# HansiZeng/scaling-retriever

Hardware: AMD Instinct MI355X
Metric: MSMARCO-Dev queries/sec end-to-end (query encode + dense brute-force top-1000) (higher is better)
Workload: dtype f32

## Files before the change

### scaling_retriever_amd/csrc/attention_f32.hip

```cpp
#include "kernels.h"
#include <math.h>

#define AF_KC 64
#define AF_RPW 4
#define AF_ROWS 16

template <int HD>
__global__ __launch_bounds__(256) void attention_f32_kernel(AttnF32Args a) {
    constexpr int DPL = HD / 64;
    __shared__ float Ks[AF_KC][HD + 1];
    __shared__ float qs[AF_ROWS][HD];
    __shared__ float ps[AF_ROWS][AF_KC];
    __shared__ unsigned char kval[AF_KC];
    const int b = blockIdx.x, h = blockIdx.y;
    const int tid = threadIdx.x, lane = tid & 63, wave = tid >> 6;
    const int t0 = a.cu_seqlens[b];
    const int S = a.cu_seqlens[b + 1] - t0;
    const int r0 = blockIdx.z * AF_ROWS;
    if (r0 >= S || S <= a.only_gt) return;
    const int G = a.nh / a.nkv, kvh = h / G;
    const int ld = (a.nh + 2 * a.nkv) * HD;
    const int koff = a.nh * HD + kvh * HD, voff = (a.nh + a.nkv) * HD + kvh * HD;
    const int nrows = (S - r0) < AF_ROWS ? (S - r0) : AF_ROWS;

// ... 102 lines not shown
#pragma unroll
            for (int e = 0; e < DPL; ++e) o[r][e] = 0.f;
        }
        for (int k0 = 0; k0 < S; k0 += AF_KC) {
            const int nk = (S - k0) < AF_KC ? (S - k0) : AF_KC;
            __syncthreads();
            for (int i = tid; i < nk * HD; i += 64 * G) {
                const int k = i / HD, d = i % HD;
                Ks[k][d] = a.qkv[(int64_t)(t0 + k0 + k) * ld + koff + d];
                if constexpr (V_LDS) Vs[k][d] = a.qkv[(int64_t)(t0 + k0 + k) * ld + voff + d];
            }
            if (tid < AF_KC) kval[tid] = (tid < nk) ? a.key_valid[t0 + k0 + tid] : 0;
            __syncthreads();
            const bool valid = kval[lane] != 0;
#pragma unroll
            for (int r = 0; r < AF_RPW; ++r) {
                const int row = rq + r;
                if (row >= nrows) break;
#pragma unroll
                for (int e = 0; e < DPL; ++e) qs[wave][lane + 64 * e] = a.qkv[(int64_t)(t0 + r0 + row) * ld + h * HD + lane + 64 * e];
                __builtin_amdgcn_wave_barrier();
                float s = 0.f;
                for (int d = 0; d < HD; ++d) s += qs[wave][d] * Ks[lane][d];
                s = valid ? s * a.scale : -INFINITY;
                float mx = s;
                for (int off = 32; off > 0; off >>= 1) mx = fmaxf(mx, __shfl_xor(mx, off));
                if (mx == -INFINITY) continue;
                const float m_new = fmaxf(m[r], mx);
                const float corr = expf(m[r] - m_new);
                const float p = valid ? expf(s - m_new) : 0.f;
                float sum = p;
                for (int off = 32; off > 0; off >>= 1) sum += __shfl_xor(sum, off);
                l[r] = l[r] * corr + sum;
                m[r] = m_new;
                ps[wave][lane] = p;
                __builtin_amdgcn_wave_barrier();
                float acc[DPL];
#pragma unroll
                for (int e = 0; e < DPL; ++e) acc[e] = 0.f;
                for (int k = 0; k < nk; ++k) {
                    const float pk = ps[wave][k];
                    if constexpr (V_LDS) {
                        acc[0] += pk * Vs[k][lane];
                    } else {
                        const float* vrow = a.qkv + (int64_t)(t0 + k0 + k) * ld + voff;
#pragma unroll
                        for (int e = 0; e < DPL; ++e) acc[e] += pk * vrow[lane + 64 * e];
                    }
                }
#pragma unroll
                for (int e = 0; e < DPL; ++e) o[r][e] = o[r][e] * corr + acc[e];
            }
        }
#pragma unroll
        for (int r = 0; r < AF_RPW; ++r) {
            const int row = rq + r;
            if (row >= nrows) break;
            const float inv = l[r] > 0.f ? 1.0f / l[r] : 0.f;
            if (a.out_f32) {
#pragma unroll
                for (int e = 0; e < DPL; ++e) a.out_f32[(int64_t)(t0 + r0 + row) * a.nh * HD + h * HD + lane + 64 * e] = o[r][e] * inv;
                continue;
            }
            bf16_t* orow = a.out + (int64_t)(t0 + r0 + row) * ldo;
#pragma unroll
            for (int e = 0; e < DPL; ++e) {
                unsigned short p[3];
                split_bf16x3(o[r][e] * inv, p[0], p[1], p[2]);
                const int col = h * HD + lane + 64 * e;
                for (int sg = 0; sg < a.out_map.n_seg; ++sg) orow[(int64_t)sg * a.nh * HD + col] = p[a.out_map.plane[sg]];
            }
        }
    }
}

template <int HD>
__global__ __launch_bounds__(256) void attention_f32_mfma_kernel(AttnF32Args a) {
    constexpr int LDK = HD + 1, CB = HD / 16;
    extern __shared__ float af_smem[];
    const int b = blockIdx.x, kvh = blockIdx.y;
    const int tid = threadIdx.x, lane = tid & 63, wave = tid >> 6;
    const int t0 = a.cu_seqlens[b];
    const int S = a.cu_seqlens[b + 1] - t0;
    if (S <= 0 || S > a.only_le) return;
    const int nkb = (S + 15) >> 4;
    const int SP = nkb * 16;
    float* Ks = af_smem;
    float* Vs = Ks + SP * LDK;
    float* Qs = Vs + SP * LDK + wave * 16 * LDK;
    const int G = a.nh / a.nkv;
    const int h = kvh * G + wave;
    const int ld = (a.nh + 2 * a.nkv) * HD;
    const int koff = a.nh * HD + kvh * HD, voff = (a.nh + a.nkv) * HD + kvh * HD;
    for (int i = tid; i < SP * (HD / 4); i += 256) {
        const int k = i / (HD / 4), d = (i % (HD / 4)) * 4;
        f32x4 kv = {0.f, 0.f, 0.f, 0.f}, vv = {0.f, 0.f, 0.f, 0.f};
        if (k < S) {
            kv = *reinterpret_cast<const f32x4*>(a.qkv + (int64_t)(t0 + k) * ld + koff + d);
            vv = *reinterpret_cast<const f32x4*>(a.qkv + (int64_t)(t0 + k) * ld + voff + d);
        }
#pragma unroll
        for (int e = 0; e < 4; ++e) { Ks[k * LDK + d + e] = kv[e]; Vs[k * LDK + d + e] = vv[e]; }
    }
    const int g = lane >> 4, c = lane & 15;
    unsigned vmask = 0;
    for (int kb = 0; kb < nkb; ++kb)
#pragma unroll
        for (int r = 0; r < 4; ++r) {
            const int key = 16 * kb + 4 * g + r;
            if (key < S && a.key_valid[t0 + key]) vmask |= 1u << (4 * kb + r);
        }
    __syncthreads();
    const int64_t ldo = (int64_t)a.out_map.n_seg * a.nh * HD;
    for (int qb = 0; qb < nkb; ++qb) {
        for (int i = lane; i < 16 * (HD / 4); i += 64) {
            const int r = i / (HD / 4), d = (i % (HD / 4)) * 4;
            f32x4 qv = {0.f, 0.f, 0.f, 0.f};
            if (16 * qb + r < S) qv = *reinterpret_cast<const f32x4*>(a.qkv + (int64_t)(t0 + 16 * qb + r) * ld + h * HD + d);
#pragma unroll
            for (int e = 0; e < 4; ++e) Qs[r * LDK + d + e] = qv[e];
        }
        __builtin_amdgcn_fence(__ATOMIC_ACQ_REL, "wavefront");
        f32x4 st[4];
        float qf[HD / 4];
#pragma unroll
        for (int kk = 0; kk < HD / 4; ++kk) qf[kk] = Qs[c * LDK + 4 * kk + g];
#pragma unroll
        for (int kb = 0; kb < 4; ++kb) {
            st[kb] = f32x4{0.f, 0.f, 0.f, 0.f};
            if (kb < nkb) {
#pragma unroll
                for (int kk = 0; kk < HD / 4; ++kk)
                    st[kb] = __builtin_amdgcn_mfma_f32_16x16x4f32(Ks[(16 * kb + c) * LDK + 4 * kk + g], qf[kk], st[kb], 0, 0, 0);
            }
        }
        float m = -INFINITY;
#pragma unroll
        for (int kb = 0; kb < 4; ++kb)
#pragma unroll
            for (int r = 0; r < 4; ++r) {
                const bool v = (vmask >> (4 * kb + r)) & 1;
                st[kb][r] = v ? st[kb][r] * a.scale : -INFINITY;
                m = fmaxf(m, st[kb][r]);
            }
        m = fmaxf(m, __shfl_xor(m, 16));
        m = fmaxf(m, __shfl_xor(m, 32));
        float sum = 0.f;
#pragma unroll
        for (int kb = 0; kb < 4; ++kb)
#pragma unroll
            for (int r = 0; r < 4; ++r) {
                const float p = (m > -INFINITY && st[kb][r] > -INFINITY) ? expf(st[kb][r] - m) : 0.f;
                st[kb][r] = p;
                sum += p;
            }
        sum += __shfl_xor(sum, 16);
        sum += __shfl_xor(sum, 32);
        const float inv = sum > 0.f ? 1.0f / sum : 0.f;
#pragma unroll
        for (int kb = 0; kb < 4; ++kb)
#pragma unroll
            for (int r = 0; r < 4; ++r) st[kb][r] *= inv;
#pragma unroll
        for (int cb = 0; cb < CB; ++cb) {
            f32x4 o = {0.f, 0.f, 0.f, 0.f};
#pragma unroll
            for (int kb = 0; kb < 4; ++kb) {
                if (kb < nkb) {
#pragma unroll
                    for (int mm = 0; mm < 4; ++mm)
                        o = __builtin_amdgcn_mfma_f32_16x16x4f32(st[kb][mm], Vs[(16 * kb + 4 * g + mm) * LDK + 16 * cb + c], o, 0, 0, 0);
                }
            }
#pragma unroll
            for (int r = 0; r < 4; ++r) {
                const int row = 16 * qb + 4 * g + r;
                if (row >= S) continue;
                const int col = h * HD + 16 * cb + c;
                if (a.out_f32) {
                    a.out_f32[(int64_t)(t0 + row) * a.nh * HD + col] = o[r];
                } else {
                    unsigned short p[3];
                    split_bf16x3(o[r], p[0], p[1], p[2]);
                    bf16_t* orow = a.out + (int64_t)(t0 + row) * ldo;
                    for (int sg = 0; sg < a.out_map.n_seg; ++sg) orow[(int64_t)sg * a.nh * HD + col] = p[a.out_map.plane[sg]];
                }
            }
        }
    }
}

template <int HD>
static int launch_attention_f32_mfma(const AttnF32Args& a, hipStream_t s) {
    const int sp = (int)ceil_div64(a.max_seqlen < 64 ? a.max_seqlen : 64, 16) * 16;
    const size_t lds = sizeof(float) * (size_t)(2 * sp + 4 * 16) * (HD + 1);
    static DeviceOnce attr_once;
    if (bool* slot = attr_once.pending()) {
        SR_CHECK_HIP(hipFuncSetAttribute(reinterpret_cast<const void*>(&attention_f32_mfma_kernel<HD>),
                                         hipFuncAttributeMaxDynamicSharedMemorySize, (int)(sizeof(float) * (2 * 64 + 64) * (HD + 1))));
        *slot = true;
    }
    const dim3 grid((unsigned)a.B, (unsigned)a.nkv), block(256);
    SR_REQUIRE(grid.y <= 65535, "attention(fp32): grid too large");
    hipLaunchKernelGGL(attention_f32_mfma_kernel<HD>, grid, block, lds, s, a);
    SR_CHECK_LAUNCH();
    return SR_OK;
}

int launch_attention_f32(const AttnF32Args& a_in, hipStream_t s) {
    AttnF32Args a = a_in;
    SR_REQUIRE(a.nh % a.nkv == 0, "attention(fp32): num_heads %d not a multiple of num_kv_heads %d", a.nh, a.nkv);
    SR_REQUIRE(a.out_f32 || (a.out_map.n_seg >= 1 && a.out_map.n_seg <= SR_MAX_SEG), "attention(fp32): bad segment map");
    if (a.B == 0 || a.max_seqlen <= 0) return SR_OK;
    const int G = a.nh / a.nkv;
    a.only_le = 0; a.only_gt = 0;
    const char* env_m = sr_dev_getenv("SR_ATTN_F32_MFMA");
    if (G == 4 && (a.hd == 64 || a.hd == 128) && !(env_m && *env_m == '0')) {
        a.only_le = 64;
        SR_TRY(a.hd == 64 ? launch_attention_f32_mfma<64>(a, s) : launch_attention_f32_mfma<128>(a, s));
        if (a.max_seqlen <= 64) return SR_OK;
        a.only_le = 0; a.only_gt = 64;
    }
    const char* env = sr_dev_getenv("SR_ATTN_F32_GQA");
    if (G == 4 && !(env && *env == '0')) {
        const dim3 grid((unsigned)a.B, (unsigned)a.nkv, (unsigned)ceil_div64(a.max_seqlen, AF_ROWS)), block(256);
        SR_REQUIRE(grid.y <= 65535 && grid.z <= 65535, "attention(fp32): grid too large");
        switch (a.hd) {
            case 64: hipLaunchKernelGGL((attention_f32_gqa_kernel<64, 4>), grid, block, 0, s, a); break;
            case 128: hipLaunchKernelGGL((attention_f32_gqa_kernel<128, 4>), grid, block, 0, s, a); break;
            default: sr_set_error("attention(fp32): head_dim %d not supported (64 or 128)", a.hd); return SR_ERR_UNSUPPORTED;
        }
        SR_CHECK_LAUNCH();
        return SR_OK;
    }
    const dim3 grid((unsigned)a.B, (unsigned)a.nh, (unsigned)ceil_div64(a.max_seqlen, AF_ROWS)), block(256);
    SR_REQUIRE(grid.y <= 65535 && grid.z <= 65535, "attention(fp32): grid too large");
    switch (a.hd) {
        case 64: hipLaunchKernelGGL(attention_f32_kernel<64>, grid, block, 0, s, a); break;
        case 128: hipLaunchKernelGGL(attention_f32_kernel<128>, grid, block, 0, s, a); break;
        default: sr_set_error("attention(fp32): head_dim %d not supported (64 or 128)", a.hd); return SR_ERR_UNSUPPORTED;
    }
    SR_CHECK_LAUNCH();
    return SR_OK;
}
```

### scaling_retriever_amd/csrc/encoder.hip

```cpp
#include "kernels.h"
#include <math.h>
#include <mutex>
#include <string>
#include <vector>

__global__ void plan_rows_kernel(const int64_t* __restrict__ mask, int B, int L, int mode, int* __restrict__ span_start,
                                 int* __restrict__ span_len, int* __restrict__ pool_start, int* __restrict__ row_len,
                                 const int* __restrict__ row_shift) {
    const int b = blockIdx.x;
    const int lane = threadIdx.x;
    int len = 0, first = L, last = -1;
    for (int p = lane; p < L; p += 64) {
        if (mask[(int64_t)b * L + p] != 0) {
            ++len;
            first = p < first ? p : first;
            last = p > last ? p : last;
        }
    }
    for (int off = 32; off > 0; off >>= 1) {
        len += __shfl_xor(len, off);
        const int f = __shfl_xor(first, off), l = __shfl_xor(last, off);
        first = f < first ? f : first;
        last = l > last ? l : last;
    }
// ... 861 lines not shown
    }
    SR_CHECK_HIP(hipDeviceSynchronize());
    m->finalized = true;
    return SR_OK;
}

extern "C" int sr_model_weight_segments(sr_model* m, int32_t* out, int64_t capacity, int64_t* n) {
    SR_REQUIRE(m && n, "sr_model_weight_segments: null argument");
    SR_REQUIRE(m->finalized, "sr_model_weight_segments: sr_model_finalize was not called");
    const sr_model_config& c = m->cfg;
    std::vector<int32_t> v;
    const bool f16p = c.fp32_planes == SR_FP32_PLANES_F16;
    const int32_t plain = c.fp32_planes ? split_map_w(c.fp32_planes).n_seg : 0;
    for (const LayerW& l : m->layers) {
        v.push_back(f16p ? l.qkv_seg : plain); v.push_back(f16p ? l.o_seg : plain);
        v.push_back(f16p ? l.gu_seg : plain); v.push_back(f16p ? l.down_seg : plain);
    }
    if (c.has_lm_head) v.push_back(f16p ? m->lm_head_seg : plain);
    *n = (int64_t)v.size();
    SR_REQUIRE(capacity >= 0 && (capacity == 0 || out), "sr_model_weight_segments: bad output buffer");
    for (int64_t i = 0; i < capacity && i < (int64_t)v.size(); ++i) out[i] = v[(size_t)i];
    return SR_OK;
}

enum { PREC_BF16 = 0, PREC_FP32 = 1 };

static int ensure_fp32_workspace(sr_model* m) {
    if (m->xs) return SR_OK;
    const sr_model_config& c = m->cfg;
    SR_REQUIRE(c.fp32_planes > 0, "encode(fp32): the model was created with fp32_planes = 0 (bf16 regime only)");
    const int64_t Tm = m->Tm, H = c.hidden_size, I = c.intermediate_size;
    const int64_t nq = (int64_t)c.num_heads * c.head_dim, nkv = (int64_t)c.num_kv_heads * c.head_dim;
    const int64_t nsg = split_map_a(c.fp32_planes).n_seg;
    auto A = [&](void** p, int64_t bytes) {
        if (hipMalloc(p, (size_t)bytes) != hipSuccess) { *p = nullptr; return false; }
        return hipMemset(*p, 0, (size_t)bytes) == hipSuccess;
    };
    const bool f16p = c.fp32_planes == SR_FP32_PLANES_F16;
    bool ok = A((void**)&m->xs, Tm * H * 2 * nsg) && A((void**)&m->qkv_f, Tm * (nq + 2 * nkv) * 4) &&
              A((void**)&m->attn_s, Tm * nq * 2 * nsg) && A((void**)&m->act_s, Tm * I * 2 * nsg);
    if (ok && f16p)
        ok = A((void**)&m->attn_f, Tm * nq * 4) && A((void**)&m->act_f, Tm * I * 4) && A((void**)&m->xs_i, Tm * 4) &&
             A((void**)&m->attn_i, Tm * 4) && A((void**)&m->act_i, Tm * 4) && A((void**)&m->act_sc, Tm * 4);
    if (!ok) {
        auto F = [](void* p) { if (p) (void)hipFree(p); };
        F(m->xs); F(m->qkv_f); F(m->attn_s); F(m->act_s); F(m->attn_f); F(m->act_f); F(m->xs_i); F(m->attn_i); F(m->act_i);
        m->xs = nullptr; m->qkv_f = nullptr; m->attn_s = nullptr; m->act_s = nullptr;
        m->attn_f = nullptr; m->act_f = nullptr; m->xs_i = nullptr; m->attn_i = nullptr; m->act_i = nullptr;
        sr_set_error("encode(fp32): hipMalloc of the fp32-regime workspace failed (%lld tokens)", (long long)Tm);
        return SR_ERR_NOMEM;
    }
    return SR_OK;
}

static int launch_rmsnorm_split(float* x, const float* embed, const int* tok_id, const float* w, bf16_t* xs, int T, int H,
                                float eps, const SplitMap& map, hipStream_t s) {
    if (T == 0) return SR_OK;
    hipLaunchKernelGGL(rmsnorm_split_kernel, dim3((unsigned)ceil_div64(T, 4)), dim3(256), 0, s, x, embed, tok_id, w, xs, T, H, eps,
                       map);
    SR_CHECK_LAUNCH();
    return SR_OK;
}

static int model_forward(sr_model* m, const int64_t* d_ids, const int64_t* d_mask, int B, int L, int mode, int prec,
                         hipStream_t s, int* T_out, const int32_t* d_shift = nullptr) {
    const sr_model_config& c = m->cfg;
    SR_REQUIRE(m->finalized, "encode: sr_model_finalize was not called");
    SR_REQUIRE(B >= 1 && L >= 1, "encode: bad batch shape [%d, %d]", B, L);
    SR_REQUIRE(B <= m->Bm, "encode: batch of %d sequences exceeds max_batch_seqs %d", B, m->Bm);
    SR_REQUIRE(L <= m->max_pos, "encode: sequence length %d exceeds %d", L, m->max_pos);
    SR_REQUIRE(d_ids && d_mask, "encode: null input");
    if (prec == PREC_FP32) SR_TRY(ensure_fp32_workspace(m));
    const int H = c.hidden_size, I = c.intermediate_size;
    const int nq = c.num_heads * c.head_dim, nkv = c.num_kv_heads * c.head_dim;

    hipLaunchKernelGGL(plan_rows_kernel, dim3(B), dim3(64), 0, s, d_mask, B, L, mode, m->span_start, m->span_len,
                       m->pool_start, m->row_len, d_shift);
    hipLaunchKernelGGL(plan_scan_kernel, dim3(1), dim3(256), 0, s, m->span_len, B, m->cu);
    SR_CHECK_LAUNCH();
    SR_CHECK_HIP(hipMemcpyAsync(m->h_cu, m->cu, (size_t)(B + 1) * 4, hipMemcpyDeviceToHost, s));
    SR_CHECK_HIP(hipStreamSynchronize(s));
    const int T = m->h_cu[B];
    int max_len = 0;
    for (int b = 0; b < B; ++b) max_len = (m->h_cu[b + 1] - m->h_cu[b]) > max_len ? (m->h_cu[b + 1] - m->h_cu[b]) : max_len;
    SR_REQUIRE(T <= m->Tm, "encode: batch packs to %d tokens, workspace holds %d (raise max_batch_tokens or split the batch)", T, m->Tm);
    *T_out = T;
    m->last_T = T;
    if (T == 0) return SR_OK;
    hipLaunchKernelGGL(plan_tokens_kernel, dim3(B), dim3(128), 0, s, d_ids, d_mask, L, m->span_start, m->cu, m->tok_id,
                       m->pos, m->key_valid, m->seq_of, c.vocab_size, mode, d_shift);
    SR_CHECK_LAUNCH();

    if (prec == PREC_FP32 && c.fp32_planes == SR_FP32_PLANES_F16) {
        auto split_rows = [&](float* src, const float* embed, const int* tok, const float* w, bf16_t* dst, float* inv, int K, int nseg) {
            launch_rows_split_h(src, embed, tok, w, dst, inv, T, K, c.rms_norm_eps, nseg, s);
        };
        const char* env_fa = sr_dev_getenv("SR_FP32_FUSED_ACT");
        const bool fused_act = m->layers[0].gu_cmax && !(env_fa && *env_fa == '0');
        for (int li = 0; li < c.num_layers; ++li) {
            LayerW& l = m->layers[li];
            split_rows(m->x, li == 0 ? m->embed : (const float*)nullptr, li == 0 ? m->tok_id : (const int*)nullptr, l.ln1, m->xs, m->xs_i, H,
                       l.qkv_seg);
            GemmArgs g{};
            g.A = m->xs; g.W = l.wqkv_s; g.M = T; g.N = nq + 2 * nkv; g.K = l.qkv_seg * H; g.C = m->qkv_f; g.a_scale = m->xs_i; g.w_scale = l.wqkv_i;
            g.pos = m->pos; g.rope_cos = m->rope_cos; g.rope_sin = m->rope_sin; g.n_rope = nq + nkv; g.head_dim = c.head_dim;
            SR_TRY(launch_gemm_bf16(EPI_QKV_ROPE_F32_H, g, s));
            AttnF32Args a{};
            a.qkv = m->qkv_f; a.out_f32 = m->attn_f; a.out = nullptr; a.cu_seqlens = m->cu; a.key_valid = m->key_valid;
            a.B = B; a.nh = c.num_heads; a.nkv = c.num_kv_heads; a.hd = c.head_dim;
            a.scale = 1.0f / sqrtf((float)c.head_dim); a.max_seqlen = max_len;
            SR_TRY(launch_attention_f32(a, s));
            split_rows(m->attn_f, nullptr, nullptr, nullptr, m->attn_s, m->attn_i, nq, l.o_seg);
            g = GemmArgs{};
            g.A = m->attn_s; g.W = l.wo_s; g.M = T; g.N = H; g.K = l.o_seg * nq; g.C = m->x; g.a_scale = m->attn_i; g.w_scale = l.wo_i;
            SR_TRY(launch_gemm_bf16(EPI_RESID_F32_H, g, s));
            if (fused_act) {
                launch_rows_split_h(m->x, nullptr, nullptr, l.ln2, m->xs, m->xs_i, T, H, c.rms_norm_eps, l.gu_seg, s, l.gu_cmax, m->act_sc,
                                    m->act_i);
                g = GemmArgs{};
                g.A = m->xs; g.W = l.wgu_s; g.M = T; g.N = 2 * I; g.K = l.gu_seg * H; g.C = m->act_s; g.a_scale = m->xs_i; g.w_scale = l.wgu_i;
                g.out_scale = m->act_sc; g.out_nseg = l.down_seg;
                SR_TRY(launch_gemm_bf16(EPI_SWIGLU_SPLIT_H, g, s));
            } else {
                split_rows(m->x, nullptr, nullptr, l.ln2, m->xs, m->xs_i, H, l.gu_seg);
                g = GemmArgs{};
                g.A = m->xs; g.W = l.wgu_s; g.M = T; g.N = 2 * I; g.K = l.gu_seg * H; g.C = m->act_f; g.a_scale = m->xs_i; g.w_scale = l.wgu_i;
                SR_TRY(launch_gemm_bf16(EPI_SWIGLU_F32_H, g, s));
                split_rows(m->act_f, nullptr, nullptr, nullptr, m->act_s, m->act_i, I, l.down_seg);
            }
            g = GemmArgs{};
            g.A = m->act_s; g.W = l.wdown_s; g.M = T; g.N = H; g.K = l.down_seg * I; g.C = m->x; g.a_scale = m->act_i; g.w_scale = l.wdown_i;
            SR_TRY(launch_gemm_bf16(EPI_RESID_F32_H, g, s));
        }
        SR_CHECK_LAUNCH();
        return SR_OK;
    }
    if (prec == PREC_FP32) {
        const SplitMap ma = split_map_a(c.fp32_planes);
        const int nsg = ma.n_seg;
        for (int li = 0; li < c.num_layers; ++li) {
            LayerW& l = m->layers[li];
            SR_TRY(launch_rmsnorm_split(m->x, li == 0 ? m->embed : (const float*)nullptr, li == 0 ? m->tok_id : (const int*)nullptr,
                                        l.ln1, m->xs, T, H, c.rms_norm_eps, ma, s));
            GemmArgs g{};
            g.A = m->xs; g.W = l.wqkv_s; g.M = T; g.N = nq + 2 * nkv; g.K = nsg * H; g.C = m->qkv_f;
            g.pos = m->pos; g.rope_cos = m->rope_cos; g.rope_sin = m->rope_sin; g.n_rope = nq + nkv; g.head_dim = c.head_dim;
            SR_TRY(launch_gemm_bf16(EPI_QKV_ROPE_F32, g, s));
            AttnF32Args a{};
            a.qkv = m->qkv_f; a.out = m->attn_s; a.cu_seqlens = m->cu; a.key_valid = m->key_valid;
            a.B = B; a.nh = c.num_heads; a.nkv = c.num_kv_heads; a.hd = c.head_dim;
            a.scale = 1.0f / sqrtf((float)c.head_dim); a.max_seqlen = max_len; a.out_map = ma;
            SR_TRY(launch_attention_f32(a, s));
            g = GemmArgs{};
            g.A = m->attn_s; g.W = l.wo_s; g.M = T; g.N = H; g.K = nsg * nq; g.C = m->x;
            SR_TRY(launch_gemm_bf16(EPI_RESID_F32, g, s));
            SR_TRY(launch_rmsnorm_split(m->x, (const float*)nullptr, (const int*)nullptr, l.ln2, m->xs, T, H, c.rms_norm_eps, ma, s));
            g = GemmArgs{};
            g.A = m->xs; g.W = l.wgu_s; g.M = T; g.N = 2 * I; g.K = nsg * H; g.C = m->act_s; g.out_map = ma;
            SR_TRY(launch_gemm_bf16(EPI_SWIGLU_SPLIT, g, s));
            g = GemmArgs{};
            g.A = m->act_s; g.W = l.wdown_s; g.M = T; g.N = H; g.K = nsg * I; g.C = m->x;
            SR_TRY(launch_gemm_bf16(EPI_RESID_F32, g, s));
        }
        return SR_OK;
    }

    SR_TRY(launch_rmsnorm(m->x, m->embed, m->tok_id, (const bf16_t*)nullptr, m->layers[0].ln1, m->xn,
                       (float*)nullptr, T, H, c.rms_norm_eps, s));
    for (int li = 0; li < c.num_layers; ++li) {
        LayerW& l = m->layers[li];
        if (li > 0) {
            SR_TRY(launch_rmsnorm(m->x, (const float*)nullptr, (const int*)nullptr,
                               (const bf16_t*)m->delta, l.ln1, m->xn, (float*)nullptr, T, H, c.rms_norm_eps, s));
        }
        GemmArgs g{};
        g.A = m->xn; g.W = l.wqkv; g.M = T; g.N = nq + 2 * nkv; g.K = H; g.C = m->qkv;
        g.pos = m->pos; g.rope_cos = m->rope_cos; g.rope_sin = m->rope_sin; g.n_rope = nq + nkv; g.head_dim = c.head_dim;
        SR_TRY(launch_gemm_bf16(EPI_QKV_ROPE, g, s));
        AttnArgs a{};
        a.qkv = m->qkv; a.out = m->attn; a.cu_seqlens = m->cu; a.pos = m->pos; a.key_valid = m->key_valid;
        a.rope_cos = m->rope_cos; a.rope_sin = m->rope_sin; a.B = B; a.nh = c.num_heads; a.nkv = c.num_kv_heads;
        a.hd = c.head_dim; a.scale = 1.0f / sqrtf((float)c.head_dim);
        a.apply_rope = 0; a.max_seqlen = max_len;
        SR_TRY(launch_attention(a, s));
        g = GemmArgs{};
        g.A = m->attn; g.W = l.wo; g.M = T; g.N = H; g.K = nq; g.C = m->delta;
        SR_TRY(launch_gemm_bf16(EPI_STORE_BF16, g, s));
        SR_TRY(launch_rmsnorm(m->x, (const float*)nullptr, (const int*)nullptr,
                           (const bf16_t*)m->delta, l.ln2, m->xn, (float*)nullptr, T, H, c.rms_norm_eps, s));
        g = GemmArgs{};
        g.A = m->xn; g.W = l.wgu; g.M = T; g.N = 2 * I; g.K = H; g.C = m->act;
        SR_TRY(launch_gemm_bf16(EPI_SWIGLU, g, s));
        g = GemmArgs{};
        g.A = m->act; g.W = l.wdown; g.M = T; g.N = H; g.K = I; g.C = m->delta;
        SR_TRY(launch_gemm_bf16(EPI_STORE_BF16, g, s));
    }
    SR_TRY(launch_rmsnorm(m->x, (const float*)nullptr, (const int*)nullptr,
                       (const bf16_t*)m->delta, (const float*)nullptr, (bf16_t*)nullptr, (float*)nullptr, T, H, c.rms_norm_eps, s));
    return SR_OK;
}

static int head_dense(sr_model* m, int B, int T, int prec, float* d_out, hipStream_t s) {
    const int H = m->cfg.hidden_size;
    if (T == 0) {
        SR_CHECK_HIP(hipMemsetAsync(d_out, 0, (size_t)B * H * 4, s));
        return SR_OK;
    }
    float2* stats = reinterpret_cast<float2*>(prec == PREC_FP32 ? (void*)m->xs : (void*)m->xn);
    hipLaunchKernelGGL(dense_head_stats_kernel, dim3((unsigned)ceil_div64(T, 4)), dim3(256), 0, s, m->x, m->norm_w, stats, T, H,
                       m->cfg.rms_norm_eps);
    hipLaunchKernelGGL(dense_head_pool_kernel, dim3((unsigned)B, (unsigned)ceil_div64(H, 256)), dim3(256), 0, s, m->x, m->norm_w,
                       stats, m->cu, m->pos, m->pool_start, d_out, H);
    SR_CHECK_LAUNCH();
    return SR_OK;
}

static int head_sparse(sr_model* m, int B, int T, int prec, float* d_out, hipStream_t s) {
    const int H = m->cfg.hidden_size, V = m->cfg.vocab_size;
    SR_CHECK_HIP(hipMemsetAsync(d_out, 0, (size_t)B * V * 4, s));
    if (T == 0) return SR_OK;
    GemmArgs g{};
    GemmEpilogue epi = EPI_SEGMAX;
    if (prec == PREC_FP32 && m->cfg.fp32_planes == SR_FP32_PLANES_F16) {
        launch_rows_split_h(m->x, (const float*)nullptr, (const int*)nullptr, (const float*)m->norm_w, m->xs, m->xs_i, T, H,
                            m->cfg.rms_norm_eps, m->lm_head_seg, s);
        g.A = m->xs; g.W = m->lm_head_s; g.K = m->lm_head_seg * H; g.a_scale = m->xs_i; g.w_scale = m->lm_head_i;
        epi = EPI_SEGMAX_H;
    } else if (prec == PREC_FP32) {
        const SplitMap ma = split_map_a(m->cfg.fp32_planes);
        SR_TRY(launch_rmsnorm_split(m->x, (const float*)nullptr, (const int*)nullptr, m->norm_w, m->xs, T, H, m->cfg.rms_norm_eps,
                                    ma, s));
        g.A = m->xs; g.W = m->lm_head_s; g.K = ma.n_seg * H;
    } else {
        SR_TRY(launch_rmsnorm(m->x, (const float*)nullptr,
                           (const int*)nullptr, (const bf16_t*)nullptr, m->norm_w, m->xn, (float*)nullptr, T, H, m->cfg.rms_norm_eps, s));
        g.A = m->xn; g.W = m->lm_head; g.K = H;
    }
    g.M = T; g.N = V; g.C = d_out; g.seq_of = m->seq_of; g.out_ld = V;
    SR_TRY(launch_gemm_bf16(epi, g, s));
    const int64_t n = (int64_t)B * V;
    hipLaunchKernelGGL(sparse_finish_kernel, dim3((unsigned)ceil_div64(n, 256)), dim3(256), 0, s, d_out, n,
                       powf((float)H, -0.25f), prec == PREC_FP32 ? 0 : 1);
    SR_CHECK_LAUNCH();
    return SR_OK;
}

static int encode_any(sr_model* m, const int64_t* d_input_ids, const int64_t* d_attention_mask, int32_t B, int32_t L, int mode,
                      int prec, float* d_dense, float* d_sparse, hipStream_t s, const int32_t* d_shift = nullptr) {
    std::lock_guard<std::mutex> lock(m->mu);
    StreamOrder::Scope in_order(m->order, s);
    int T = 0;
    SR_TRY(model_forward(m, d_input_ids, d_attention_mask, B, L, mode, prec, s, &T, d_shift));
    if (mode != 1) SR_TRY(head_dense(m, B, T, prec, d_dense, s));
    if (mode != 0) SR_TRY(head_sparse(m, B, T, prec, d_sparse, s));
    return SR_OK;
}

static int encode_dense(sr_model* m, const int64_t* d_input_ids, const int64_t* d_attention_mask, int32_t B, int32_t L, int prec,
                        float* d_out, hipStream_t s) {
    return encode_any(m, d_input_ids, d_attention_mask, B, L, 0, prec, d_out, nullptr, s);
}

static int encode_sparse(sr_model* m, const int64_t* d_input_ids, const int64_t* d_attention_mask, int32_t B, int32_t L, int prec,
                         float* d_out, hipStream_t s) {
    return encode_any(m, d_input_ids, d_attention_mask, B, L, 1, prec, nullptr, d_out, s);
}

extern "C" int sr_encode_dense(sr_model* m, const int64_t* d_input_ids, const int64_t* d_attention_mask, int32_t B, int32_t L,
                               float* d_out, sr_stream stream) {
    SR_REQUIRE(m && d_out, "sr_encode_dense: null argument");
    return encode_dense(m, d_input_ids, d_attention_mask, B, L, PREC_BF16, d_out, (hipStream_t)stream);
}

extern "C" int sr_encode_dense_fp32(sr_model* m, const int64_t* d_input_ids, const int64_t* d_attention_mask, int32_t B, int32_t L,
                                    float* d_out, sr_stream stream) {
    SR_REQUIRE(m && d_out, "sr_encode_dense_fp32: null argument");
    return encode_dense(m, d_input_ids, d_attention_mask, B, L, PREC_FP32, d_out, (hipStream_t)stream);
}

extern "C" int sr_encode_sparse(sr_model* m, const int64_t* d_input_ids, const int64_t* d_attention_mask, int32_t B, int32_t L,
                                float* d_out, sr_stream stream) {
    SR_REQUIRE(m && d_out, "sr_encode_sparse: null argument");
    SR_REQUIRE(m->cfg.has_lm_head, "sr_encode_sparse: model was created without an lm_head (LlamaBiModel)");
    return encode_sparse(m, d_input_ids, d_attention_mask, B, L, PREC_BF16, d_out, (hipStream_t)stream);
}

extern "C" int sr_encode_sparse_fp32(sr_model* m, const int64_t* d_input_ids, const int64_t* d_attention_mask, int32_t B, int32_t L,
                                     float* d_out, sr_stream stream) {
    SR_REQUIRE(m && d_out, "sr_encode_sparse_fp32: null argument");
    SR_REQUIRE(m->cfg.has_lm_head, "sr_encode_sparse_fp32: model was created without an lm_head (LlamaBiModel)");
    return encode_sparse(m, d_input_ids, d_attention_mask, B, L, PREC_FP32, d_out, (hipStream_t)stream);
}

extern "C" int sr_encode_both(sr_model* m, const int64_t* d_input_ids, const int64_t* d_attention_mask, int32_t B, int32_t L,
                              int32_t fp32, float* d_out_sparse, float* d_out_dense, sr_stream stream) {
    SR_REQUIRE(m && d_out_sparse && d_out_dense, "sr_encode_both: null argument");
    SR_REQUIRE(m->cfg.has_lm_head, "sr_encode_both: model was created without an lm_head (LlamaBiModel)");
    return encode_any(m, d_input_ids, d_attention_mask, B, L, 2, fp32 ? PREC_FP32 : PREC_BF16, d_out_dense, d_out_sparse,
                      (hipStream_t)stream);
}

extern "C" int sr_encode_rows(sr_model* m, const int64_t* d_input_ids, const int64_t* d_attention_mask, int32_t B, int32_t L,
                              const int32_t* d_row_shift, int32_t mode, int32_t fp32, float* d_out_sparse, float* d_out_dense,
                              sr_stream stream) {
    SR_REQUIRE(m, "sr_encode_rows: null model");
    SR_REQUIRE(mode >= 0 && mode <= 2, "sr_encode_rows: mode %d (0 dense, 1 sparse, 2 both)", mode);
    SR_REQUIRE(mode == 1 || d_out_dense, "sr_encode_rows: null dense output");
    SR_REQUIRE(mode == 0 || d_out_sparse, "sr_encode_rows: null sparse output");
    SR_REQUIRE(mode == 0 || m->cfg.has_lm_head, "sr_encode_rows: model was created without an lm_head (LlamaBiModel)");
// ... 54 lines not shown
```

### scaling_retriever_amd/csrc/gemm_bf16.hip

```cpp
#include "kernels.h"
#include <math.h>
#include <stdlib.h>
#include <string.h>
#include <type_traits>

typedef __bf16 mfma_bf16x8 __attribute__((ext_vector_type(8)));
typedef _Float16 mfma_f16x8 __attribute__((ext_vector_type(8)));
template <bool F16>
__device__ __forceinline__ f32x4 sr_mma(const mfma_bf16x8& w, const mfma_bf16x8& a, const f32x4& c) {
    if constexpr (F16)
        return __builtin_amdgcn_mfma_f32_16x16x32_f16(__builtin_bit_cast(mfma_f16x8, w), __builtin_bit_cast(mfma_f16x8, a), c, 0, 0, 0);
    else
        return __builtin_amdgcn_mfma_f32_16x16x32_bf16(w, a, c, 0, 0, 0);
}
__device__ __forceinline__ f32x4 sr_rope_lo(const f32x4& x1, const f32x4& x2, const f32x4& c, const f32x4& s) {
#pragma clang fp contract(off)
    f32x4 y;
#pragma unroll
    for (int r = 0; r < 4; ++r) { const float a = x1[r] * c[r], b = x2[r] * s[r]; y[r] = a - b; }
    return y;
}
__device__ __forceinline__ f32x4 sr_rope_hi(const f32x4& x1, const f32x4& x2, const f32x4& c, const f32x4& s) {
#pragma clang fp contract(off)
    f32x4 y;
// ... 864 lines not shown

template <int EPI, int WAVES_N, int WAVES_M, int NB, int MB, bool PIPE = false, int NS = 2, int KL = 0>
static int launch_cfg(const GemmArgs& g_in, hipStream_t s) {
    constexpr int BN = 16 * NB * WAVES_N, BM = 16 * MB * WAVES_M;
    constexpr size_t lds = NS * (size_t)(BN + BM) * 128 + (KL == 1 ? 4 * 8192 : 0);
    static DeviceOnce attr_once;
    bool* attr_slot = attr_once.pending();
    if (attr_slot) {
        SR_CHECK_HIP(hipFuncSetAttribute(reinterpret_cast<const void*>(&gemm_bf16_kernel<EPI, WAVES_N, WAVES_M, NB, MB, PIPE, NS, KL>),
                                         hipFuncAttributeMaxDynamicSharedMemorySize, (int)lds));
        *attr_slot = true;
    }
    GemmArgs g = g_in;
    g.m_fastest = ((int64_t)g.N * g.K * 2 > (128ll << 20) && (int64_t)g.N > 4 * (int64_t)g.M) ? 1 : 0;
    if (const char* e = sr_dev_getenv("SR_GEMM_MFAST")) g.m_fastest = atoi(e);
    g.xcd_order = 1;
    if (const char* e = sr_dev_getenv("SR_GEMM_XCD")) g.xcd_order = atoi(e);
    int64_t tiles = ceil_div64(g.N, BN) * ceil_div64(g.M, BM);
    const char* env = sr_dev_getenv("SR_GEMM_PERSIST");
    constexpr int64_t by_lds = (160 * 1024) / lds;
    const int64_t slots = 256 * (WAVES_N * WAVES_M == 4 ? (by_lds > 3 ? 3 : by_lds) : (WAVES_N * WAVES_M == 1 ? (by_lds > 8 ? 8 : by_lds) : 1));
    if (!(env && *env == '0') && tiles > slots) tiles = slots;
    hipLaunchKernelGGL((gemm_bf16_kernel<EPI, WAVES_N, WAVES_M, NB, MB, PIPE, NS, KL>), dim3((unsigned)tiles), dim3(64 * WAVES_N * WAVES_M), lds,
                       s, g);
    SR_CHECK_LAUNCH();
    return SR_OK;
}

static double plan_cost(int64_t big_tiles, int64_t small_tiles) {
    double c = (double)ceil_div64(big_tiles, 256);
    if (small_tiles > 0) {
        const int64_t full = small_tiles / 512, rest = small_tiles % 512;
        c += 0.61 * (double)full + (rest == 0 ? 0.0 : (rest <= 256 ? 0.45 : 0.61));
        c += 0.03;
    }
    return c;
}

static int plan_big_rows(const GemmArgs& g, bool small_allowed) {
    const char* env = sr_dev_getenv("SR_GEMM_TILE");
    if (env && *env) {
        if (atoi(env) == 256) return g.M;
        if (atoi(env) == 128) return 0;
        if (!strncmp(env, "split:", 6)) {
            const int rows = atoi(env + 6) / 256 * 256;
            return rows < g.M ? rows : g.M;
        }
    }
    if (!small_allowed) return g.M;
    const int64_t tn256 = ceil_div64(g.N, 256), tn128 = ceil_div64(g.N, 128);
    int best_rows = 0;
    double best = plan_cost(0, tn128 * ceil_div64(g.M, 128));
    if (tn256 * ceil_div64(g.M, 256) >= 128) {
        const double all_big = plan_cost(tn256 * ceil_div64(g.M, 256), 0);
        if (all_big <= best) { best = all_big; best_rows = g.M; }
        for (int rows = 256; rows < g.M; rows += 256) {
            const double c = plan_cost(tn256 * (rows / 256), tn128 * ceil_div64(g.M - rows, 128));
            if (c < best - 1e-9) { best = c; best_rows = rows; }
        }
    }
    return best_rows;
}

template <int EPI>
static int launch_big(const GemmArgs& g, hipStream_t s) {
    if constexpr (EPI == EPI_STORE_BF16 || EPI == EPI_SWIGLU || EPI == EPI_QKV_ROPE) {
        const char* big = sr_dev_getenv("SR_GEMM_BIG");
        if (big && big[0] == 's' && big[1] == '3' && g.K / G_BK >= 4) {
            if constexpr (EPI == EPI_QKV_ROPE) {
                if (g.head_dim == 64) return launch_cfg<EPI, 2, 4, 8, 2, true, 3>(g, s);
            } else {
                return launch_cfg<EPI, 2, 4, 8, 2, true, 3>(g, s);
            }
        }
    }
    const char* env = sr_dev_getenv("SR_GEMM_PIPE");
    {
        const char* big = sr_dev_getenv("SR_GEMM_BIG");
        const bool want8 = big && big[0] == '8', want4 = big && big[0] == '4';
        constexpr bool STAGED_BF16 = EPI == EPI_STORE_BF16 || EPI == EPI_SWIGLU || EPI == EPI_STORE_F32 || EPI == EPI_RESID_F32 || EPI == EPI_QKV_ROPE;
        constexpr bool STAGED_F16 = EPI == EPI_RESID_F32_H || EPI == EPI_SWIGLU_SPLIT_H;
        if constexpr (STAGED_BF16 || STAGED_F16) {
            const bool rope_ok = EPI != EPI_QKV_ROPE || g.n_rope % 128 == 0;
            if (g.K / G_BK >= 4 && (int64_t)g.K * 512 < (1ll << 31) && !want8 && (STAGED_BF16 || want4) && rope_ok && !(env && *env == '0'))
                return launch_cfg<EPI, 2, 2, 8, 8, true, 2, 1>(g, s);
        }
    }
    if (g.K / G_BK >= 4 && !(env && *env == '0')) return launch_cfg<EPI, 2, 4, 8, 4, true>(g, s);
    return launch_cfg<EPI, 2, 4, 8, 4, false>(g, s);
}

static bool env_off(const char* name) {
    const char* e = sr_dev_getenv(name);
    return e && *e == '0';
}

template <int EPI>
static int launch_small(const GemmArgs& g, hipStream_t s) {
    const bool pipe = g.K / G_BK >= 4 && !env_off("SR_GEMM_PIPE");
    if constexpr (EPI == EPI_QKV_ROPE || EPI == EPI_QKV_ROPE_F32 || EPI == EPI_QKV_ROPE_F32_H) {
        if (g.head_dim == 128) return launch_cfg<EPI, 1, 4, 8, 2>(g, s);
    }
    if constexpr (EPI != EPI_QKV_ROPE && EPI != EPI_QKV_ROPE_F32 && EPI != EPI_QKV_ROPE_F32_H) {
        const int64_t t128 = ceil_div64(g.N, 128) * ceil_div64(g.M, 128);
        if (t128 < 384 && g.M > 64 && !env_off("SR_GEMM_TAIL64"))
            return pipe ? (env_off("SR_GEMM_NS3") ? launch_cfg<EPI, 2, 2, 4, 2, true>(g, s) : launch_cfg<EPI, 2, 2, 4, 2, true, 3>(g, s))
                        : launch_cfg<EPI, 2, 2, 4, 2>(g, s);
    }
    return pipe ? launch_cfg<EPI, 2, 2, 4, 4, true>(g, s) : launch_cfg<EPI, 2, 2, 4, 4>(g, s);
}

template <int EPI>
static GemmArgs rows_from(const GemmArgs& g, int row0) {
    GemmArgs t = g;
    t.A = g.A + (int64_t)row0 * g.K;
    t.M = g.M - row0;
    const int64_t ldc = (EPI == EPI_SWIGLU || EPI == EPI_SWIGLU_F32 || EPI == EPI_SWIGLU_F32_H)
                            ? g.N / 2 : (EPI == EPI_SWIGLU_SPLIT ? (int64_t)g.out_map.n_seg * (g.N / 2) : (EPI == EPI_SWIGLU_SPLIT_H ? (int64_t)g.out_nseg * (g.N / 2) : g.N));
    const int64_t esz = (EPI == EPI_STORE_F32 || EPI == EPI_RESID_F32 || EPI == EPI_QKV_ROPE_F32 || EPI == EPI_SWIGLU_F32 ||
                         (EPI >= EPI_H_FIRST && EPI != EPI_SWIGLU_SPLIT_H)) ? 4 : 2;
    if constexpr (EPI != EPI_SEGMAX && EPI != EPI_SEGMAX_H) t.C = reinterpret_cast<unsigned char*>(g.C) + (int64_t)row0 * ldc * esz;
    if (g.a_scale) t.a_scale = g.a_scale + row0;
    if (g.out_scale) t.out_scale = g.out_scale + row0;
    if (g.seq_of) t.seq_of = g.seq_of + row0;
    if (g.pos) t.pos = g.pos + row0;
    t.stamps = nullptr;
    return t;
}

static int skinny_max_rows() {
    const char* e = sr_dev_getenv("SR_GEMM_SKINNY");
    if (!e || !*e) return 64;
    return atoi(e);
}

template <int EPI>
static int launch_one(const GemmArgs& g, hipStream_t s) {
    if constexpr (EPI == EPI_QKV_ROPE || EPI == EPI_QKV_ROPE_F32 || EPI == EPI_QKV_ROPE_F32_H) {
        SR_REQUIRE(g.head_dim == 64 || g.head_dim == 128, "gemm(qkv+rope): head_dim %d not supported", g.head_dim);
        SR_REQUIRE(g.pos && g.rope_cos && g.rope_sin && g.n_rope % g.head_dim == 0 && g.n_rope <= g.N && g.N % g.head_dim == 0,
                   "gemm(qkv+rope): bad rope arguments");
    }
    if (g.M <= skinny_max_rows() && g.K / G_BK >= 4) {
        if (g.M > 32) {
            if constexpr (EPI == EPI_QKV_ROPE || EPI == EPI_QKV_ROPE_F32 || EPI == EPI_QKV_ROPE_F32_H) {
                if (g.head_dim == 128) return launch_cfg<EPI, 1, 1, 8, 4, true, 3>(g, s);
            }
            return launch_cfg<EPI, 1, 1, 4, 4, true, 4>(g, s);
        }
        if (g.M > 16) {
            if constexpr (EPI == EPI_QKV_ROPE || EPI == EPI_QKV_ROPE_F32 || EPI == EPI_QKV_ROPE_F32_H) {
                if (g.head_dim == 128) return launch_cfg<EPI, 1, 1, 8, 2, true, 4>(g, s);
            }
            return launch_cfg<EPI, 1, 1, 4, 2, true, 4>(g, s);
        }
        if constexpr (EPI == EPI_QKV_ROPE || EPI == EPI_QKV_ROPE_F32 || EPI == EPI_QKV_ROPE_F32_H) {
            if (g.head_dim == 128) return launch_cfg<EPI, 1, 1, 8, 1, true, 4>(g, s);
        }
        return launch_cfg<EPI, 1, 1, 4, 1, true, 4>(g, s);
    }
    {
        const int big_rows = plan_big_rows(g, true);
        if (big_rows >= g.M) return launch_big<EPI>(g, s);
        if (big_rows <= 0) return launch_small<EPI>(g, s);
        GemmArgs head = g;
        head.M = big_rows;
        SR_TRY(launch_big<EPI>(head, s));
// ... 38 lines not shown
```

### scaling_retriever_amd/csrc/kernels.h

```cpp
#pragma once
#include "common.h"

typedef unsigned short bf16_t;

enum GemmEpilogue {
    EPI_STORE_BF16 = 0,
    EPI_RESID_F32 = 1,
    EPI_SWIGLU = 2,
    EPI_SEGMAX = 3,
    EPI_STORE_F32 = 4,
    EPI_QKV_ROPE = 5,
    EPI_QKV_ROPE_F32 = 6,
    EPI_SWIGLU_SPLIT = 7,
    EPI_SWIGLU_F32 = 8,
    EPI_H_FIRST = 9,
    EPI_QKV_ROPE_F32_H = 9, EPI_RESID_F32_H = 10, EPI_SWIGLU_F32_H = 11, EPI_SEGMAX_H = 12,
    EPI_SWIGLU_SPLIT_H = 13,
    EPI_SWIGLU_SPLITH_BASE = 14,
};

#define SR_MAX_SEG 6
struct SplitMap {
    int n_seg;
    int plane[SR_MAX_SEG];
};
#define SR_FP32_PLANES_F16 16
inline SplitMap split_map_a(int planes) {
    if (planes == 3) return SplitMap{6, {2, 0, 1, 1, 0, 0}};
    return SplitMap{3, {1, 0, 0, 0, 0, 0}};
}
inline SplitMap split_map_w(int planes) {
    if (planes == 3) return SplitMap{6, {0, 2, 1, 0, 1, 0}};
    return SplitMap{3, {0, 1, 0, 0, 0, 0}};
}

struct GemmArgs {
    const bf16_t* A;
    const bf16_t* W;
    int M, N, K;
    void* C;
    const int* seq_of;
    int64_t out_ld;
    const int* pos;
    const float* rope_cos;
    const float* rope_sin;
    int n_rope;
    int head_dim;
    unsigned long long* stamps;
    const float* a_scale;
    const float* w_scale;
    const float* out_scale;
    int out_nseg;
    SplitMap out_map;
    int m_fastest;
    int xcd_order;
};

int launch_gemm_bf16(GemmEpilogue epi, const GemmArgs& g, hipStream_t s);

struct AttnArgs {
    const bf16_t* qkv;
    bf16_t* out;
    const int* cu_seqlens;
    const int* pos;
    const unsigned char* key_valid;
    const float* rope_cos;
    const float* rope_sin;
    int B, nh, nkv, hd;
    float scale;
    int apply_rope;
    int max_seqlen;
};
int launch_attention(const AttnArgs& a, hipStream_t s);

struct AttnF32Args {
    const float* qkv;
    float* out_f32;
    bf16_t* out;
    const int* cu_seqlens;
    const unsigned char* key_valid;
    int B, nh, nkv, hd;
    float scale;
    int max_seqlen;
    SplitMap out_map;
    int only_le = 0, only_gt = 0;
};
int launch_attention_f32(const AttnF32Args& a, hipStream_t s);
```

Baseline: 16020.

## Bucket short sequences into 16-token length classes for MFMA attention; widen staged GEMM tile

```diff
diff --git a/scaling_retriever_amd/csrc/attention_f32.hip b/scaling_retriever_amd/csrc/attention_f32.hip
--- a/scaling_retriever_amd/csrc/attention_f32.hip
+++ b/scaling_retriever_amd/csrc/attention_f32.hip
@@ -208,7 +208,7 @@
     const int tid = threadIdx.x, lane = tid & 63, wave = tid >> 6;
     const int t0 = a.cu_seqlens[b];
     const int S = a.cu_seqlens[b + 1] - t0;
-    if (S <= 0 || S > a.only_le) return;
+    if (S <= a.only_gt || S > a.only_le) return;
     const int nkb = (S + 15) >> 4;
     const int SP = nkb * 16;
     float* Ks = af_smem;
@@ -318,7 +318,7 @@
 
 template <int HD>
 static int launch_attention_f32_mfma(const AttnF32Args& a, hipStream_t s) {
-    const int sp = (int)ceil_div64(a.max_seqlen < 64 ? a.max_seqlen : 64, 16) * 16;
+    const int sp = (int)ceil_div64(a.only_le, 16) * 16;
     const size_t lds = sizeof(float) * (size_t)(2 * sp + 4 * 16) * (HD + 1);
     static DeviceOnce attr_once;
     if (bool* slot = attr_once.pending()) {
@@ -342,8 +342,18 @@
     a.only_le = 0; a.only_gt = 0;
     const char* env_m = sr_dev_getenv("SR_ATTN_F32_MFMA");
     if (G == 4 && (a.hd == 64 || a.hd == 128) && !(env_m && *env_m == '0')) {
-        a.only_le = 64;
-        SR_TRY(a.hd == 64 ? launch_attention_f32_mfma<64>(a, s) : launch_attention_f32_mfma<128>(a, s));
+        const char* env_c = sr_dev_getenv("SR_ATTN_F32_CLASSES");
+        const int top = a.max_seqlen < 64 ? a.max_seqlen : 64;
+        if (env_c && *env_c == '0') {
+            a.only_le = (int)ceil_div64(top, 16) * 16;
+            SR_TRY(a.hd == 64 ? launch_attention_f32_mfma<64>(a, s) : launch_attention_f32_mfma<128>(a, s));
+        } else {
+            for (int c = 1; 16 * (c - 1) < top; ++c) {
+                if (a.len_classes && !((a.len_classes >> (c - 1)) & 1u)) continue;
+                a.only_gt = 16 * (c - 1); a.only_le = 16 * c;
+                SR_TRY(a.hd == 64 ? launch_attention_f32_mfma<64>(a, s) : launch_attention_f32_mfma<128>(a, s));
+            }
+        }
         if (a.max_seqlen <= 64) return SR_OK;
         a.only_le = 0; a.only_gt = 64;
     }
diff --git a/scaling_retriever_amd/csrc/encoder.hip b/scaling_retriever_amd/csrc/encoder.hip
--- a/scaling_retriever_amd/csrc/encoder.hip
+++ b/scaling_retriever_amd/csrc/encoder.hip
@@ -967,7 +967,12 @@
     SR_CHECK_HIP(hipStreamSynchronize(s));
     const int T = m->h_cu[B];
     int max_len = 0;
-    for (int b = 0; b < B; ++b) max_len = (m->h_cu[b + 1] - m->h_cu[b]) > max_len ? (m->h_cu[b + 1] - m->h_cu[b]) : max_len;
+    unsigned len_classes = 0;
+    for (int b = 0; b < B; ++b) {
+        const int len = m->h_cu[b + 1] - m->h_cu[b];
+        max_len = len > max_len ? len : max_len;
+        if (len >= 1 && len <= 64) len_classes |= 1u << ((len - 1) >> 4);
+    }
     SR_REQUIRE(T <= m->Tm, "encode: batch packs to %d tokens, workspace holds %d (raise max_batch_tokens or split the batch)", T, m->Tm);
     *T_out = T;
     m->last_T = T;
@@ -987,34 +992,34 @@
             split_rows(m->x, li == 0 ? m->embed : (const float*)nullptr, li == 0 ? m->tok_id : (const int*)nullptr, l.ln1, m->xs, m->xs_i, H,
                        l.qkv_seg);
             GemmArgs g{};
-            g.A = m->xs; g.W = l.wqkv_s; g.M = T; g.N = nq + 2 * nkv; g.K = l.qkv_seg * H; g.C = m->qkv_f; g.a_scale = m->xs_i; g.w_scale = l.wqkv_i;
+            g.A = m->xs; g.W = l.wqkv_s; g.M = T; g.N = nq + 2 * nkv; g.K = l.qkv_seg * H; g.a_nseg = l.qkv_seg; g.C = m->qkv_f; g.a_scale = m->xs_i; g.w_scale = l.wqkv_i;
             g.pos = m->pos; g.rope_cos = m->rope_cos; g.rope_sin = m->rope_sin; g.n_rope = nq + nkv; g.head_dim = c.head_dim;
             SR_TRY(launch_gemm_bf16(EPI_QKV_ROPE_F32_H, g, s));
             AttnF32Args a{};
             a.qkv = m->qkv_f; a.out_f32 = m->attn_f; a.out = nullptr; a.cu_seqlens = m->cu; a.key_valid = m->key_valid;
             a.B = B; a.nh = c.num_heads; a.nkv = c.num_kv_heads; a.hd = c.head_dim;
-            a.scale = 1.0f / sqrtf((float)c.head_dim); a.max_seqlen = max_len;
+            a.scale = 1.0f / sqrtf((float)c.head_dim); a.max_seqlen = max_len; a.len_classes = len_classes;
             SR_TRY(launch_attention_f32(a, s));
             split_rows(m->attn_f, nullptr, nullptr, nullptr, m->attn_s, m->attn_i, nq, l.o_seg);
             g = GemmArgs{};
-            g.A = m->attn_s; g.W = l.wo_s; g.M = T; g.N = H; g.K = l.o_seg * nq; g.C = m->x; g.a_scale = m->attn_i; g.w_scale = l.wo_i;
+            g.A = m->attn_s; g.W = l.wo_s; g.M = T; g.N = H; g.K = l.o_seg * nq; g.a_nseg = l.o_seg; g.C = m->x; g.a_scale = m->attn_i; g.w_scale = l.wo_i;
             SR_TRY(launch_gemm_bf16(EPI_RESID_F32_H, g, s));
             if (fused_act) {
                 launch_rows_split_h(m->x, nullptr, nullptr, l.ln2, m->xs, m->xs_i, T, H, c.rms_norm_eps, l.gu_seg, s, l.gu_cmax, m->act_sc,
                                     m->act_i);
                 g = GemmArgs{};
-                g.A = m->xs; g.W = l.wgu_s; g.M = T; g.N = 2 * I; g.K = l.gu_seg * H; g.C = m->act_s; g.a_scale = m->xs_i; g.w_scale = l.wgu_i;
+                g.A = m->xs; g.W = l.wgu_s; g.M = T; g.N = 2 * I; g.K = l.gu_seg * H; g.a_nseg = l.gu_seg; g.C = m->act_s; g.a_scale = m->xs_i; g.w_scale = l.wgu_i;
                 g.out_scale = m->act_sc; g.out_nseg = l.down_seg;
                 SR_TRY(launch_gemm_bf16(EPI_SWIGLU_SPLIT_H, g, s));
             } else {
                 split_rows(m->x, nullptr, nullptr, l.ln2, m->xs, m->xs_i, H, l.gu_seg);
                 g = GemmArgs{};
-                g.A = m->xs; g.W = l.wgu_s; g.M = T; g.N = 2 * I; g.K = l.gu_seg * H; g.C = m->act_f; g.a_scale = m->xs_i; g.w_scale = l.wgu_i;
+                g.A = m->xs; g.W = l.wgu_s; g.M = T; g.N = 2 * I; g.K = l.gu_seg * H; g.a_nseg = l.gu_seg; g.C = m->act_f; g.a_scale = m->xs_i; g.w_scale = l.wgu_i;
                 SR_TRY(launch_gemm_bf16(EPI_SWIGLU_F32_H, g, s));
                 split_rows(m->act_f, nullptr, nullptr, nullptr, m->act_s, m->act_i, I, l.down_seg);
             }
             g = GemmArgs{};
-            g.A = m->act_s; g.W = l.wdown_s; g.M = T; g.N = H; g.K = l.down_seg * I; g.C = m->x; g.a_scale = m->act_i; g.w_scale = l.wdown_i;
+            g.A = m->act_s; g.W = l.wdown_s; g.M = T; g.N = H; g.K = l.down_seg * I; g.a_nseg = l.down_seg; g.C = m->x; g.a_scale = m->act_i; g.w_scale = l.wdown_i;
             SR_TRY(launch_gemm_bf16(EPI_RESID_F32_H, g, s));
         }
         SR_CHECK_LAUNCH();
@@ -1034,7 +1039,7 @@
             AttnF32Args a{};
             a.qkv = m->qkv_f; a.out = m->attn_s; a.cu_seqlens = m->cu; a.key_valid = m->key_valid;
             a.B = B; a.nh = c.num_heads; a.nkv = c.num_kv_heads; a.hd = c.head_dim;
-            a.scale = 1.0f / sqrtf((float)c.head_dim); a.max_seqlen = max_len; a.out_map = ma;
+            a.scale = 1.0f / sqrtf((float)c.head_dim); a.max_seqlen = max_len; a.len_classes = len_classes; a.out_map = ma;
             SR_TRY(launch_attention_f32(a, s));
             g = GemmArgs{};
             g.A = m->attn_s; g.W = l.wo_s; g.M = T; g.N = H; g.K = nsg * nq; g.C = m->x;
@@ -1109,7 +1114,7 @@
     if (prec == PREC_FP32 && m->cfg.fp32_planes == SR_FP32_PLANES_F16) {
         launch_rows_split_h(m->x, (const float*)nullptr, (const int*)nullptr, (const float*)m->norm_w, m->xs, m->xs_i, T, H,
                             m->cfg.rms_norm_eps, m->lm_head_seg, s);
-        g.A = m->xs; g.W = m->lm_head_s; g.K = m->lm_head_seg * H; g.a_scale = m->xs_i; g.w_scale = m->lm_head_i;
+        g.A = m->xs; g.W = m->lm_head_s; g.K = m->lm_head_seg * H; g.a_nseg = m->lm_head_seg; g.a_scale = m->xs_i; g.w_scale = m->lm_head_i;
         epi = EPI_SEGMAX_H;
     } else if (prec == PREC_FP32) {
         const SplitMap ma = split_map_a(m->cfg.fp32_planes);
diff --git a/scaling_retriever_amd/csrc/gemm_bf16.hip b/scaling_retriever_amd/csrc/gemm_bf16.hip
--- a/scaling_retriever_amd/csrc/gemm_bf16.hip
+++ b/scaling_retriever_amd/csrc/gemm_bf16.hip
@@ -970,7 +970,7 @@
         constexpr bool STAGED_F16 = EPI == EPI_RESID_F32_H || EPI == EPI_SWIGLU_SPLIT_H;
         if constexpr (STAGED_BF16 || STAGED_F16) {
             const bool rope_ok = EPI != EPI_QKV_ROPE || g.n_rope % 128 == 0;
-            if (g.K / G_BK >= 4 && (int64_t)g.K * 512 < (1ll << 31) && !want8 && (STAGED_BF16 || want4) && rope_ok && !(env && *env == '0'))
+            if (g.K / G_BK >= 4 && (int64_t)g.K * 512 < (1ll << 31) && !want8 && (STAGED_BF16 || want4 || g.a_nseg == 2) && rope_ok && !(env && *env == '0'))
                 return launch_cfg<EPI, 2, 2, 8, 8, true, 2, 1>(g, s);
         }
     }
diff --git a/scaling_retriever_amd/csrc/kernels.h b/scaling_retriever_amd/csrc/kernels.h
--- a/scaling_retriever_amd/csrc/kernels.h
+++ b/scaling_retriever_amd/csrc/kernels.h
@@ -50,6 +50,7 @@
     const float* a_scale;
     const float* w_scale;
     const float* out_scale;
+    int a_nseg;
     int out_nseg;
     SplitMap out_map;
     int m_fastest;
@@ -84,5 +85,6 @@
     int max_seqlen;
     SplitMap out_map;
     int only_le = 0, only_gt = 0;
+    unsigned len_classes = 0;
 };
 int launch_attention_f32(const AttnF32Args& a, hipStream_t s);
```

Result: faster. 16200, median of 6 (+1.1%).
